# sriramelango/optimized-diffusion-model

Hardware: AMD Instinct MI355X
Metric: trajectories/sec (1000-step PC sampler, NCSN++ [1,9,9], bs=128/GPU) (higher is better)
Workload: dtype f32; 1 GPU; NCSN++ nf=64 ch_mult=[1,2,2] on [128,1,9,9] per GPU, 1000-step reflected PC sampler (predictor euler_maruyama, corrector none), classifier-free guidance on (2B-sample forwards), fp32; global_batch=128, num_scales=1000, score_evals_per_traj=999, parallelism=single GPU

## Files before the change

### optimized-diffusion-model_amd/csrc/rdmi.hip

```cpp
#include <hip/hip_runtime.h>

#include <algorithm>
#include <cmath>
#include <cstdarg>
#include <cstdio>
#include <cstdlib>
#include <cstring>
#include <climits>
#include <map>
#include <memory>
#include <stdexcept>
#include <string>
#include <vector>

#include "../../include/rdmi.h"
#include "attn_kernel.h"
#include "conv_kernel.h"
#include "misc_kernels.h"
#include "unet_kernel.h"
#include "bwd_kernels.h"
#include "opt_kernels.h"
#include "ode_kernels.h"
#include "tiled_kernels.h"

// ... 270 lines not shown
    }
    add_conv_p(c, "input_conv", a.channels, a.nf);
    for (auto& b : L.down) add_resblock_p(c, b.name, b.cin, b.cout);
    for (size_t i = 0; i < L.down.size(); ++i)
        if (L.down[i].attn) add_attn_p(c, "down_attn." + std::to_string(i), L.down[i].cout);
    {
        int ch = a.nf;
        for (int i = 0; i < a.n_levels; ++i) {
            ch = a.nf * a.ch_mult[i];
            if (i != a.n_levels - 1) add_conv_p(c, "downsample." + std::to_string(i) + ".Conv_0", ch, ch);
        }
    }
    add_resblock_p(c, "mid_block1", L.mid_ch, L.mid_ch);
    add_resblock_p(c, "mid_block2", L.mid_ch, L.mid_ch);
    for (auto& b : L.up) add_resblock_p(c, b.name, b.cin, b.cout);
    for (size_t i = 0; i < L.up.size(); ++i)
        if (L.up[i].attn) add_attn_p(c, "up_attn." + std::to_string(i), L.up[i].cout);
    for (int k = 0, i = a.n_levels - 1; i >= 1; --i, ++k) {
        const int ch = a.nf * a.ch_mult[i];
        add_conv_p(c, "upsample." + std::to_string(k) + ".Conv_0", ch, ch);
    }
    add_gn(c, "out_norm", a.nf * a.ch_mult[0]);
    add_conv_p(c, "out_conv", a.nf * a.ch_mult[0], a.channels);
}

inline bool up_fold_shape_ok(int Hs, int Ws, int Cin, int Cout) {
    return std::getenv("RDMI_NO_UP_FOLD") == nullptr && Hs * Ws == 16 && Cin == Cout && Cin % 128 == 0;
}

inline bool k_fold_shape_ok(int C, int L) {
    return std::getenv("RDMI_NO_K_FOLD") == nullptr && std::getenv("RDMI_NO_ATTN_FOLD") == nullptr && std::getenv("RDMI_NO_QKV1") == nullptr && C == 64 && L <= 96;
}

struct Builder {
    rdmi_ctx* c;
    std::vector<int> ints;
    size_t wf = 0;

    int new_tensor(const std::string& name, int C, int H, int W) {
        Tensor t;
        t.name = name; t.C = C; t.H = H; t.W = W;
        t.def = (int)c->ops.size();
        c->tensors.push_back(t);
        return (int)c->tensors.size() - 1;
    }
    void use(int t) { if (t >= 0) c->tensors[t].last = (int)c->ops.size(); }

    size_t alloc_w(size_t n) { size_t o = wf; wf += (n + 63) & ~(size_t)63; return o; }

    void job_pack(const std::string& pname, size_t dst_off, int Cin, int Cout, int Kpad, int Npad, int n_off, int ntap,
                  long s_co, long s_ci, long s_t) {
        PackJob j{};
        j.dst = reinterpret_cast<float*>(dst_off);
        j.Cin = Cin; j.Cout = Cout; j.Kpad = Kpad; j.Npad = Npad; j.n_off = n_off; j.ntap = ntap;
        j.s_co = s_co; j.s_ci = s_ci; j.s_t = s_t; j.kind = 0;
        c->jobs.push_back(j);
        c->job_param.push_back(c->pindex.at(pname));
    }
    void job_copy(const std::string& pname, size_t dst_off, int n, int n_off) {
        PackJob j{};
        j.dst = reinterpret_cast<float*>(dst_off);
        j.Cout = n; j.n_off = n_off; j.kind = 1;
        c->jobs.push_back(j);
        c->job_param.push_back(c->pindex.at(pname));
    }
    size_t pack_conv(const std::string& pre, int cin, int cout) {
// ... 600 lines not shown
            const BlockSpec& bs = L.up[u];
            HS sk = hs.back();
            hs.pop_back();
            const int Hs = H, Ws = W;
            H = sk.H; W = sk.W;
            h = add_resblock(b, bs.name, h, sk.t, ch, sk.C, Hs, Ws, H, W, bs.cout, dense_off[bs.name], &err);
            if (err) return err;
            ch = bs.cout;
            if (bs.attn) { h = b.add_attn("up_attn." + std::to_string(u), h, ch, H, W, &err); if (err) return err; }
        }
        if (k != a.n_levels - 1) {
            ConvSpec s;
            s.name = "upsample." + std::to_string(k);
            s.tA = h; s.CA = ch; s.Ha = H; s.Wa = W; s.Hv = 2 * H; s.Wv = 2 * W;
            s.conv = s.name + ".Conv_0"; s.Ho = 2 * H; s.Wo = 2 * W; s.Cout = ch;
            h = b.add_conv(s, &err);
            if (err) return err;
            if (k == a.n_levels - 2 && up_fold_shape_ok(H, W, ch, ch)) {
                const int Kp = pad16(ch), Np = pad16(ch);
                const size_t o = b.alloc_w((size_t)16 * Kp * Np);
                b.job_pack(s.conv + ".weight", o, ch, ch, Kp, Np, 0, 16, (long)ch * 9, 9, 1);
                c->jobs.back().kind = 5;
                c->wmap[s.conv + ".up4"] = o;
            }
            H *= 2; W *= 2;
        }
    }
    if (H != c->H || W != c->W) return fail("network output grid %dx%d != input %dx%d", H, W, c->H, c->W);
    ConvSpec out;
    out.name = "out_conv"; out.tA = h; out.CA = ch; out.Ha = H; out.Wa = W; out.Hv = H; out.Wv = W;
    out.gn = "out_norm"; out.conv = "out_conv"; out.Ho = H; out.Wo = W; out.Cout = a.channels; out.to_output = true;
    b.add_conv(out, &err);
    if (err) return err;

    {
        struct Blk { size_t off, size; };
        std::vector<Blk> freel;
        std::vector<std::vector<int>> dies((size_t)c->ops.size() + 1);
        for (size_t t = 0; t < c->tensors.size(); ++t) {
            Tensor& tt = c->tensors[t];
            if (tt.last < tt.def) tt.last = tt.def;
            dies[(size_t)tt.last].push_back((int)t);
        }
        size_t top = 0;
        size_t ti = 0;
        for (size_t o = 0; o < c->ops.size(); ++o) {
            for (; ti < c->tensors.size() && c->tensors[ti].def == (int)o; ++ti) {
                Tensor& tt = c->tensors[ti];
                const size_t need = (tt.per_sample() + 63) & ~(size_t)63;
                int best = -1;
                if (!c->debug_taps)
                    for (size_t f = 0; f < freel.size(); ++f)
                        if (freel[f].size >= need && (best < 0 || freel[f].size < freel[(size_t)best].size)) best = (int)f;
                if (best >= 0) {
                    tt.off = freel[(size_t)best].off;
                    if (freel[(size_t)best].size > need) { freel[(size_t)best].off += need; freel[(size_t)best].size -= need; }
                    else freel.erase(freel.begin() + best);
                } else { tt.off = top; top += need; }
            }
            for (int t : dies[o]) {
                const Tensor& tt = c->tensors[(size_t)t];
                freel.push_back({tt.off, (tt.per_sample() + 63) & ~(size_t)63});
            }
        }
        c->ws_per_sample = top;
    }
// ... 155 lines not shown
        for (int p = 0; p < 4; ++p)
            for (int y = 0; y < Hs; ++y)
                for (int x = 0; x < Ws; ++x) {
                    const int sy = y + (tap >> 1) - 1 + (p >> 1), sx = x + (tap & 1) - 1 + (p & 1);
                    if (sy >= 0 && sy < Hs && sx >= 0 && sx < Ws) v[(size_t)p * Hs * Ws + y * Ws + x] = (short)(sy * Ws + sx);
                }
        char key[64];
        snprintf(key, sizeof key, "up4:%d,%d,%d", Hs, Ws, tap);
        return add_table(key, v);
    }

    FOp blank(int kind) {
        FOp o;
        std::memset(&o, 0, sizeof o);
        o.kind = kind; o.a_off = -1; o.b_off = -1; o.a_map_off = -1; o.dense_off = -1; o.resid_off = -1; o.scale = 1.f; o.src_off = -1; o.gn_off = -1; o.samp = cur_samp; o.drop_op = -1;
        return o;
    }
    int emit(const FOp& o) { flush_xchg(); prog.fprog.push_back(o); return (int)prog.fprog.size() - 1; }
    int emit_xchg(const LT& t, const LT* own_rows_src) {
        FOp o = blank(FOP_XCHG);
        o.dst_off = t.off; o.dst_rs = t.rs; o.xidx = n_xchg++;
        if (own_rows_src) {
            o.a_hw = 1; o.rows = own_rows_src->hw(); o.C = t.C; o.a_off = own_rows_src->off; o.a_rs = own_rows_src->rs;
            if (own_rows_src->C != t.C || t.rows() != 4 * o.rows) fail_("exchange: row-slice shapes");
        } else {
            o.a_hw = 0; o.rows = t.rows(); o.C = t.C / 4;
        }
        if (o.C < 32 || o.C > 128 || (o.C & (o.C - 1)) || o.rows * o.C > 512) fail_("exchange: block of " + std::to_string(o.rows) + " x " + std::to_string(o.C));
        xslot_granules = std::max(xslot_granules, 2 * o.rows * o.C);
        prog.fprog.push_back(o);
        return (int)prog.fprog.size() - 1;
    }
    void flush_xchg() { if (pendx.on) { pendx.on = false; emit_xchg(pendx.t, nullptr); } }
    enum { F_GAMMA, F_BETA, F_BIAS, F_BIAS2, F_W, F_SC0W, F_SC1W, F_BIAS_ARENA };
    void patch_param(int op, int field, const std::string& param) { prog.fpatch.push_back({op, field, param, 0}); }
    void patch_arena(int op, int field, size_t off) { prog.fpatch.push_back({op, field, "", off}); }

    void gather_x(const LT& dst) {
        FOp o = blank(FOP_GATHER);
        o.dst_off = dst.off; o.dst_rs = dst.rs; o.rows = dst.rows(); o.C = dst.C;
        o.CA = c->arch.channels; o.CB = 0; o.a_off = -2; o.a_hw = dst.hw(); o.hw_shift = shift_of(dst.hw());
        emit(o);
    }
    void gather_g(const LT& dst, size_t spill) {
        FOp o = blank(FOP_GATHER);
        o.dst_off = dst.off; o.dst_rs = dst.rs; o.rows = dst.rows(); o.C = dst.C;
        o.CA = dst.C; o.CB = 0; o.a_off = -1; o.a_hw = dst.hw(); o.a_mod = 0; o.hw_shift = shift_of(dst.hw());
        const int idx = emit(o);
        spill_fix.push_back({idx, spill, 2});
    }
    void gather_cat(const LT& dst, const LT& A, size_t spillB, int CB) {
        FOp o = blank(FOP_GATHER);
        o.dst_off = dst.off; o.dst_rs = dst.rs; o.rows = dst.rows(); o.C = dst.C;
        o.CA = A.C; o.CB = CB; o.a_off = A.off; o.a_rs = A.rs; o.a_hw = A.hw(); o.hw_shift = shift_of(dst.hw());
        if (A.H != dst.H || A.W != dst.W || A.pm) o.a_map_off = map_table(A.H, A.W, dst.H, dst.W, A.pm);
        if (A.pm && A.ns != 1) fail_("phase-major tensors are single-sample");
        o.b_off = -1;
        const int idx = emit(o);
        spill_fix.push_back({idx, spillB, 1});
    }
    void copy_t(const LT& dst, const LT& src) {
        if (src.pm) fail_("copy of a phase-major tensor");
        FOp o = blank(FOP_GATHER);
        o.dst_off = dst.off; o.dst_rs = dst.rs; o.rows = dst.rows(); o.C = dst.C;
        o.CA = src.C; o.CB = 0; o.a_off = src.off; o.a_rs = src.rs; o.a_hw = src.hw(); o.hw_shift = shift_of(dst.hw());
        emit(o);
    }
    struct SpillFix { int op; size_t off; int which; };
    std::vector<size_t> slot_log; size_t slot_pos = 0; bool slot_replay = false;
    std::vector<SpillFix> spill_fix;
    size_t spill_store(const LT& t) {
        if (t.pm) fail_("spill of a phase-major tensor");
        FOp o = blank(FOP_STORE);
        o.dst_off = t.off; o.dst_rs = t.rs; o.rows = t.rows(); o.C = t.C; o.hw_shift = shift_of(t.hw());
// ... 110 lines not shown
                }
            }
            prog.fprog[(size_t)idx].drop_op = -1;
        }
        if (coop && cur_samp < 0) {
            FOp& q = prog.fprog[(size_t)idx];
            q.coop = 1;
            if (q.Cout_pad != 128 || q.mtiles != 1 || q.main_ph.nch % 4 != 0 || dst_kind != 0 || !dst || dst->C != 128)
                fail_("co-operative conv shape (Cout " + std::to_string(Cout) + ", " + std::to_string(q.mtiles) + " row tiles, " + std::to_string(q.main_ph.nch) + " chunks)");
            if (ntap == 9) { pendx.on = true; pendx.t = *dst; }
        }
        return idx;
    }
    bool up_fold_ok(const LT& in, int Hv, int Wv, int Cout) const {
        return !train && cur_samp >= 0 && !in.pm && Hv == 2 * in.H && Wv == 2 * in.W && up_fold_shape_ok(in.H, in.W, in.C, Cout) &&
               c->wmap.count("upsample." + std::to_string(c->arch.n_levels - 2) + ".Conv_0.up4") != 0;
    }
    int conv_up4(const LT& in, const std::string& wkey, int Cout, const std::string& bias_param, LT* dst) {
        FOp o = blank(FOP_CONV);
        o.rows = 4 * in.hw(); o.mtiles = 4; o.Cout = Cout; o.Cout_pad = pad16(Cout);
        o.ntap = 4; o.hw_shift = shift_of(o.rows);
        o.main_ph.lds_off = in.off; o.main_ph.rs = in.rs; o.main_ph.nch = in.C / 16;
        for (int t = 0; t < 4; ++t) o.tab_off[t] = up4_table(in.H, in.W, t);
        o.w_tile_stride = 4 * in.C * o.Cout_pad * (int)sizeof(float);
        o.dst_off = dst->off; o.dst_rs = dst->rs;
        if (o.main_ph.nch % 8 != 0 || o.rows <= 4 || o.dst_kind != 0 || in.C != Cout || in.hw() != 16 || in.pm || cur_samp < 0 || dst->C != Cout || dst->hw() != o.rows)
            fail_("folded upsample conv: unsupported shape (" + std::to_string(in.H) + "x" + std::to_string(in.W) + " source, " + std::to_string(in.C) + " -> " + std::to_string(Cout) + " channels)");
        dst->pm = true;
        const int idx = emit(o);
        patch_arena(idx, F_W, c->wmap.at(wkey + ".up4"));
        patch_param(idx, F_BIAS, bias_param);
        return idx;
    }
};

FusedBuilder::LT fused_resblock(FusedBuilder& b, const std::string& name, FusedBuilder::LT& xin, int cout, int dense_off) {
    using LT = FusedBuilder::LT;
    const int H = xin.H, W = xin.W;
    const float rs2 = (float)(1.0 / std::sqrt(2.0));
    if (xin.C != cout) {
        LT out = b.talloc(cout, H, W);
        b.conv(xin, H, W, H, W, 1, 0, 1, name + ".NIN_0", 0, cout, name + ".NIN_0.b", 0, 0, &out, 1.f, -1, nullptr, nullptr, "", "");
        b.gn(xin, name + ".GroupNorm_0", true);
        LT h1 = b.talloc(cout, H, W);
        b.conv(xin, H, W, H, W, 1, 1, 9, name + ".Conv_0", 0, cout, name + ".Conv_0.bias", 0, 0, &h1, 1.f, dense_off, nullptr, nullptr, "", "");
        b.tfree(xin);
        b.gn(h1, name + ".GroupNorm_1", true);
        b.conv(h1, H, W, H, W, 1, 1, 9, name + ".Conv_1", 0, cout, name + ".Conv_1.bias", 0, 0, &out, rs2, -1, &out, nullptr, "", "");
        b.tfree(h1);
        return out;
    }
    LT xact = b.talloc(xin.C, H, W);
    b.gn(xact, name + ".GroupNorm_0", true, &xin);
    LT h1 = b.talloc(cout, H, W);
    b.conv(xact, H, W, H, W, 1, 1, 9, name + ".Conv_0", 0, cout, name + ".Conv_0.bias", 0, 0, &h1, 1.f, dense_off, nullptr, nullptr, "", "");
    b.tfree(xact);
    b.gn(h1, name + ".GroupNorm_1", true);
    LT out = b.talloc(cout, H, W);
    b.conv(h1, H, W, H, W, 1, 1, 9, name + ".Conv_1", 0, cout, name + ".Conv_1.bias", 0, 0, &out, rs2, -1, &xin, nullptr, "", "");
    b.tfree(h1);
    b.tfree(xin);
    return out;
}

FusedBuilder::LT fused_attn(FusedBuilder& b, const std::string& name, FusedBuilder::LT& x) {
    using LT = FusedBuilder::LT;
// ... 93 lines not shown
        for (size_t i = 0; i < c->ops.size(); ++i) b.lp_op[c->ops[i].name] = (int)i;
    }
    const int nslot0 = coop ? 1 : S;
    Layout L = build_layout(c);
    std::map<std::string, int> dense_off;
    {
        int dt = 0;
        for (auto& d : L.down) { dense_off[d.name] = dt; dt += d.cout; }
        dense_off["mid_block1"] = dt; dt += L.mid_ch;
        dense_off["mid_block2"] = dt; dt += L.mid_ch;
        for (auto& u : L.up) { dense_off[u.name] = dt; dt += u.cout; }
    }
    const int zero_bytes = 1280;
    const int stat_bytes = 1024 + 64;
    b.arena_init(TAB_RESERVE + zero_bytes + stat_bytes);
    b.gn_slot_off = TAB_RESERVE + zero_bytes;
    b.gn_fuse = std::getenv("RDMI_NO_GNFUSE") == nullptr;
    const int H0 = c->H, W0 = c->W;
    if (H0 * W0 > 96) { q.why = "more than 96 pixels per sample"; return 0; }
    const int nlev = a.n_levels;
    const bool multi = S > 1;

    struct HS { size_t spill; int C, H, W; };
    std::vector<HS> hs;
    int ch = a.nf, H = H0, W = W0;
    size_t hand_down = 0, hand_up = 0;
    LT h;
    const int nrb = a.num_res_blocks;
    for (int sl = 0; sl < nslot0; ++sl) {
        b.cur_samp = sl;
        b.slot_replay = sl > 0; b.slot_pos = 0;
        H = H0; W = W0; ch = a.nf;
        LT xin = b.talloc(16, H, W);
        b.gather_x(xin);
        h = b.talloc(a.nf, H, W);
        b.conv(xin, H, W, H, W, 1, 1, 9, "input_conv", 0, a.nf, "input_conv.bias", 0, 0, &h, 1.f, -1, nullptr, nullptr, "", "");
        b.tfree(xin);
        if (sl == 0) hs.push_back({(size_t)-1, a.nf, H, W});
        for (int j = 0; j < nrb; ++j) {
            const BlockSpec& bs = L.down[(size_t)j];
            h = fused_resblock(b, bs.name, h, bs.cout, dense_off[bs.name]);
            ch = bs.cout;
            if (bs.attn) h = fused_attn(b, "down_attn." + std::to_string(j), h);
            const size_t sp = b.spill_store(h);
            if (sl == 0) hs.push_back({sp, ch, H, W});
        }
        if (sl == 0) hs.push_back(hs.back());
        if (nlev > 1) {
            const int Ho = (H + 1 - 3) / 2 + 1, Wo = (W + 1 - 3) / 2 + 1;
            LT o = b.talloc(ch, Ho, Wo);
            const std::string nm = "downsample.0.Conv_0";
            b.conv(h, H, W, Ho, Wo, 2, 0, 9, nm, 0, ch, nm + ".bias", 0, 0, &o, 1.f, -1, nullptr, nullptr, "", "");
            b.tfree(h);
            h = o; H = Ho; W = Wo;
            if (multi && !coop) { hand_down = b.spill_store(h); b.tfree(h); }
        }
    }
    b.slot_replay = false;
    int d = nrb, u = 0, loadtab_idx = -1;
    {
        b.cur_samp = (multi && !coop) ? -1 : 0;
        int loadtab_op = -1;
        bool in_coop = false;
        auto enter_multi = [&]() {
            b.multi_slot_off = b.alloc_top(4096);
            b.tab1_lds = b.alloc_top(TAB1_RESERVE);
            FOp lt = b.blank(FOP_LOADTAB);
            lt.dst_off = b.tab1_lds;
            loadtab_op = b.emit(lt);
// ... 78 lines not shown
        if (multi && !coop) {
            hand_up = b.spill_store(h); b.tfree(h);
            leave_multi();
        }
        loadtab_idx = loadtab_op;
    }
    const int u0 = u, ch_low = ch, H_low = H, W_low = W;
    const std::vector<HS> hs0 = hs;
    for (int sl = 0; sl < nslot0; ++sl) {
        b.cur_samp = sl;
        u = u0; ch = ch_low; H = H_low; W = W_low; hs = hs0;
        if (multi && !coop) { h = b.talloc(ch, H, W); b.gather_g(h, hand_up); }
        if (nlev > 1) {
            LT o = b.talloc(ch, 2 * H, 2 * W);
            const std::string nm = "upsample." + std::to_string(nlev - 2) + ".Conv_0";
            if (b.up_fold_ok(h, 2 * H, 2 * W, ch)) b.conv_up4(h, nm, ch, nm + ".bias", &o);
            else b.conv(h, 2 * H, 2 * W, 2 * H, 2 * W, 1, 1, 9, nm, 0, ch, nm + ".bias", 0, 0, &o, 1.f, -1, nullptr, nullptr, "", "");
            b.tfree(h);
            h = o; H *= 2; W *= 2;
        }
        for (int j = 0; j < nrb + 1; ++j, ++u) {
            const BlockSpec& bs = L.up[(size_t)u];
            HS sk = hs.back();
            hs.pop_back();
            LT cat = b.talloc(ch + sk.C, sk.H, sk.W);
            b.gather_cat(cat, h, sk.spill, sk.C);
            b.tfree(h);
            H = sk.H; W = sk.W;
            h = fused_resblock(b, bs.name, cat, bs.cout, dense_off[bs.name]);
            ch = bs.cout;
            if (bs.attn) h = fused_attn(b, "up_attn." + std::to_string(u), h);
        }
        b.gn(h, "out_norm", true);
        b.conv(h, H, W, H, W, 1, 1, 9, "out_conv", 0, a.channels, "out_conv.bias", 0, 2, nullptr, 1.f, -1, nullptr, nullptr, "", "");
        b.tfree(h);
    }
    if (H != c->H || W != c->W) b.fail_("network output grid differs from the input grid");

    *tab_used = (int)q.ftabs.size() * 2 + 16;
    *tab1_used = (int)b.tabs1.size() * 2 + 16;
    if (*tab_used > TAB_RESERVE && TAB_RESERVE != 8 * 1024) b.fail_("row tables exceed the reserved LDS region");
    if (*tab1_used > TAB1_RESERVE && multi) b.fail_("low-resolution row tables exceed their LDS block");
    int cmax = 16;
    for (auto& o : q.fprog) if (o.kind == FOP_CONV) { cmax = std::max(cmax, o.main_ph.nch * 16); for (int s2 = 0; s2 < o.nsc; ++s2) cmax = std::max(cmax, o.sc[s2].nch * 16); }
    if (cmax * 4 + 64 > zero_bytes) b.fail_("zero row too small");
    if (b.failed && TAB_RESERVE == 8 * 1024 && *tab_used <= 8 * 1024) return 0;
    if (b.failed) { q.why = b.why; return 0; }

    auto tab_lds = [&](int ref) { return (ref >> 24) ? b.tab1_lds + (ref & 0xffffff) * 2 : (ref & 0xffffff) * 2; };
    for (auto& o : q.fprog) {
        if (o.kind == FOP_CONV) {
            for (int t = 0; t < o.ntap; ++t) o.tab_off[t] = tab_lds(o.tab_off[t]);
            for (int s2 = 0; s2 < o.nsc; ++s2) o.sc[s2].tab_off = tab_lds(o.sc[s2].tab_off);
        } else if (o.kind == FOP_GATHER && o.a_map_off >= 0) {
            o.a_map_off = tab_lds(o.a_map_off);
        }
    }
    while (q.ftabs.size() % 8) q.ftabs.push_back(-1);
    const size_t tab0_shorts = q.ftabs.size();
    q.ftabs.insert(q.ftabs.end(), b.tabs1.begin(), b.tabs1.end());
    q.spill_per_sample = b.spill_floats;
    int coop_max_nb = 0, spill_n = c->max_batch;
    if (coop) {
        const int st = c->coop_stride, res = resident_workgroups();
        const int max_groups = (res / (4 * st)) * st;
        coop_max_nb = std::min(c->max_batch, 4 * max_groups);
        if (coop_max_nb < 1) b.fail_("no room for one co-operative group");
        const int grid_max = ceil_div(ceil_div(std::max(coop_max_nb, 1), 4), st) * 4 * st;
        spill_n = 4 * grid_max;
    }
    if (b.failed) { q.why = b.why; return 0; }
    HIP_OK(hip_alloc(q.d_spill, std::max<size_t>(q.spill_per_sample, 1) * (size_t)spill_n));
    HIP_OK(hip_alloc(q.d_fprog, q.fprog.size()));
    HIP_OK(hip_alloc(q.d_ftabs, q.ftabs.size()));
    HIP_OK(hipMemcpy(q.d_ftabs.get(), q.ftabs.data(), q.ftabs.size() * sizeof(short), hipMemcpyHostToDevice));
    for (auto& f : b.spill_fix) {
        FOp& o = q.fprog[(size_t)f.op];
        float* p = q.d_spill.get() + f.off * (size_t)spill_n;
        if (f.which == 1) o.b_g = p; else if (f.which == 2) o.a_g = p; else o.g_out = p;
    }
    UnetArgs& fa = q.fargs;
    fa = UnetArgs{};
    fa.prog = q.d_fprog.get(); fa.nops = (int)q.fprog.size();
    fa.tabs = q.d_ftabs.get(); fa.tab_bytes = (int)(tab0_shorts * sizeof(short)); fa.tab_base = 0;
    if (loadtab_idx >= 0) q.fprog[(size_t)loadtab_idx].a_g = reinterpret_cast<const float*>(q.d_ftabs.get() + tab0_shorts);
    fa.zero_off = TAB_RESERVE; fa.zero_bytes = zero_bytes;
// ... 129 lines not shown
    }
    HIP_OK(hipGetLastError());
    for (auto& op : c->ops) {
        if (op.kind == OP_CONV) {
            ConvArgs& a = op.conv;
            a.bias = P(c, op.p_bias);
            a.bias_sc = op.p_bias_sc.empty() ? nullptr : P(c, op.p_bias_sc);
            a.gamma = op.p_gamma.empty() ? nullptr : P(c, op.p_gamma);
            a.beta = op.p_beta.empty() ? nullptr : P(c, op.p_beta);
        } else {
            op.attn.gamma = P(c, op.p_gamma); op.attn.beta = P(c, op.p_beta); op.attn.b3 = P(c, op.p_b3);
        }
    }
    for (auto& l : c->tl) {
        if (l.kind == 6) { l.gact.gamma = P(c, l.p_gamma); l.gact.beta = P(c, l.p_beta); continue; }
        if (l.kind != 0) continue;
        l.conv.bias = l.p_bias.empty() ? c->d_w.get() + l.bias_arena : P(c, l.p_bias);
        l.conv.gamma = l.p_gamma.empty() ? nullptr : P(c, l.p_gamma);
        l.conv.beta = l.p_beta.empty() ? nullptr : P(c, l.p_beta);
    }
    for (auto& q : c->progs) {
        if (!q.ok) continue;
        for (auto& f : q.fpatch) {
            FOp& o = q.fprog[(size_t)f.op];
            const float* p = f.param.empty() ? c->d_w.get() + f.arena_off : P(c, f.param);
            switch (f.field) {
                case FusedBuilder::F_GAMMA: o.gamma = p; break;
                case FusedBuilder::F_BETA: o.beta = p; break;
                case FusedBuilder::F_BIAS: case FusedBuilder::F_BIAS_ARENA: o.bias = p; break;
                case FusedBuilder::F_BIAS2: o.bias2 = p; break;
                case FusedBuilder::F_W: o.main_ph.w = p; break;
                case FusedBuilder::F_SC0W: o.sc[0].w = p; break;
                case FusedBuilder::F_SC1W: o.sc[1].w = p; break;
            }
        }
        HIP_OK(hipMemcpyAsync(q.d_fprog.get(), q.fprog.data(), q.fprog.size() * sizeof(FOp), hipMemcpyHostToDevice, s));
    }
    if (c->fused_ready()) HIP_OK(hipStreamSynchronize(s));
    c->packed_valid = true;
    return 0;
}

struct FwdIn {
    const float* x; int x_mod;
    const float* sig; int sig_mod;
    float t_scalar;
    int t_is_time; float smin, ratio;
    const float* labels; int label_rows;
    float* out; int NB;
    const float* tt_row = nullptr;
    const float* dense_rows = nullptr;
};

int run_forward(rdmi_ctx* c, const FwdIn& f, hipStream_t s) {
    const rdmi_arch& a = c->arch;
    if (f.NB < 1 || f.NB > c->max_batch) return fail("batch %d outside [1, %d] (rdmi_create max_batch)", f.NB, c->max_batch);
    if (a.scale_by_sigma && !c->tiled) return fail("scale_by_sigma=True is only built for the tiled plan (the shipped GTO-Halo config sets it False, RD/configs/model/ncsnpp.yaml)");
    if (a.conditional && !f.labels) return fail("class_labels is required: the model is conditional (label_emb) -- reference raises here too (RD/models/ncsnpp.py:262)");
    const int T = c->temb, Np_t = (T + 63) & ~63, Np_d = (c->dense_total + 63) & ~63;
    if (!f.tt_row && !f.dense_rows) {
    LinArgs l{};
    l.M = f.NB; l.fourW = P(c, "time_embed.W"); l.nfour = a.nf;
    l.X = f.sig; l.x_mod = f.sig_mod > 0 ? f.sig_mod : f.NB; l.t_is_time = f.t_is_time; l.smin = f.smin; l.ratio = f.ratio;
    l.use_scalar = f.sig ? 0 : 1; l.t_scalar = f.t_scalar;
    l.pre = 2; l.K = pad16(2 * a.nf); l.W = c->d_w.get() + c->w_t0; l.Npad = Np_t; l.N = T; l.bias = P(c, "time_mlp.0.bias");
    l.Y = c->d_h1.get(); l.ldy = T;
// ... 862 lines not shown
```

### optimized-diffusion-model_amd/csrc/unet_kernel.h

```cpp
#pragma once
#include <cstddef>

#include "common.h"

#define UW_THREADS 512
#define UW_WAVES 8
#ifndef UW_PF_M4
#define UW_PF_M4 4
#endif
#ifndef UW_PF_N1
#define UW_PF_N1 4
#endif
#ifndef UW_PF_KS1
#define UW_PF_KS1 4
#endif
#ifndef UW_PRIO
#define UW_PRIO 0
#endif
#ifndef UW_LIGHT_BARRIER
#define UW_LIGHT_BARRIER 0
#endif

__device__ __forceinline__ void lds_barrier() {
#if defined(__HIP_DEVICE_COMPILE__) && UW_LIGHT_BARRIER
// ... 19 lines not shown
    int CA, CB;
    int a_off, a_rs, a_hw, a_mod, a_map_off;
    int b_off, b_rs;
    const float* a_g; const float* b_g;
    float* g_out;
    int G, act; float eps;
    int src_off, src_rs;
    int logT, Cg, magic_c4n, magic_Cg; float inv_cnt;
    int logG;
    const float* gamma; const float* beta;
    int ntap; int tab_off[9];
    FPhase main_ph;
    int nsc; FPhase sc[2];
    int mtiles, Cout, Cout_pad;
    const float* bias; const float* bias2;
    int dense_off;
    int resid_off, resid_rs;
    float scale;
    int dst_kind;
    int dst2_off, dst3_off, dst3_rs, split_C;
    int q_off, k_off, vt_off, p_off, qk_rs, ps;
    int L, Lpad; float att_scale;
    int gn_off, gn_rs, gn_act, gn_raw, gn_slot_off, gn_nslots;
    int samp, hw_shift;
    int qkv1;
    int coop;
    int a_mstride;
    int xidx;
    float* stash;
    int stash_bf16;
    int drop_op;
    int w_tile_stride;
    int k_rs;
};

struct UnetArgs {
    const FOp* prog; int nops;
    const short* tabs; int tab_bytes;
    int tab_base;
    int zero_off;
    int zero_bytes;
    const float* dense; int dense_stride;
    const float* x_in; int x_mod;
    float* out;
    int NB;
    int S;
    int dbg;
    long long* stamps;
    int coop, coop_stride;
    unsigned long long* xbuf;
    int xslot;
    unsigned epoch_base;
    int out_elems;
    float drop_p; const unsigned long long* seed_dev;
    int* coop_err;
    int coop_break;
};

struct OpW { int w0, w1; };
static_assert(sizeof(FOp) <= 512, "FOp must fit two VGPRs per wave");
__device__ __forceinline__ int opw_at(const OpW& r, int word) {
    return word < 64 ? __builtin_amdgcn_readlane(r.w0, word) : __builtin_amdgcn_readlane(r.w1, word - 64);
}
#define OPI(r, field) opw_at(r, (int)(offsetof(FOp, field) / 4))
#define OPF(r, field) __builtin_bit_cast(float, OPI(r, field))
#define OPP(r, T, field) \
    reinterpret_cast<T*>((unsigned long long)(unsigned)opw_at(r, (int)(offsetof(FOp, field) / 4)) | ((unsigned long long)(unsigned)opw_at(r, (int)(offsetof(FOp, field) / 4) + 1) << 32))
__device__ __forceinline__ OpW opw_load(const FOp* op, int lane) {
    OpW r;
    constexpr int NW = (int)(sizeof(FOp) / 4);
    const int* g = reinterpret_cast<const int*>(op);
    r.w0 = lane < NW ? __builtin_bit_cast(int, ldg1(reinterpret_cast<const float*>(g + lane))) : 0;
    r.w1 = lane + 64 < NW ? __builtin_bit_cast(int, ldg1(reinterpret_cast<const float*>(g + lane + 64))) : 0;
    return r;
}

__device__ __forceinline__ float* lds_f(int off) { return reinterpret_cast<float*>(rdmi_lds + off); }

__device__ __forceinline__ int samp_of(int samp, int hw_shift, int row) { return samp >= 0 ? samp : (row >> hw_shift); }

template <bool MS>
__device__ __forceinline__ void fop_gather(const OpW& w, const UnetArgs& u, int n0, int ncap, int member, int tid) {
    struct { int C, rows, dst_off, dst_rs, CA, CB, a_off, a_rs, a_hw, a_mod, a_map_off, b_off, b_rs, samp, hw_shift; const float* a_g; const float* b_g; } o;
    o.C = OPI(w, C); o.rows = OPI(w, rows); o.dst_off = OPI(w, dst_off); o.dst_rs = OPI(w, dst_rs); o.CA = OPI(w, CA); o.CB = OPI(w, CB);
    o.a_off = OPI(w, a_off); o.a_rs = OPI(w, a_rs); o.a_hw = OPI(w, a_hw); o.a_mod = OPI(w, a_mod); o.a_map_off = OPI(w, a_map_off);
    if (MS && o.a_off >= 0) o.a_off += member * OPI(w, a_mstride);
    o.b_off = OPI(w, b_off); o.b_rs = OPI(w, b_rs); o.a_g = OPP(w, const float, a_g); o.b_g = OPP(w, const float, b_g);
    o.samp = MS ? OPI(w, samp) : 0; o.hw_shift = MS ? OPI(w, hw_shift) : 0;
    const int Cd = o.C;
    const int c4n = Cd >> 2;
    const int total = o.rows * c4n;
    float* dst = lds_f(o.dst_off);
    const short* map = o.a_map_off >= 0 ? reinterpret_cast<const short*>(rdmi_lds + o.a_map_off) : nullptr;
    const int dpv = UW_THREADS / c4n, dc4 = UW_THREADS - dpv * c4n;
    int row = tid / c4n, c4 = tid - row * c4n;
    const bool from_x = o.a_off == -2;
    const float* ag = from_x ? u.x_in : o.a_g;
    const int amod = from_x ? u.x_mod : o.a_mod;
    const int hw = o.samp >= 0 ? o.rows : (1 << o.hw_shift);
    for (int i = tid; i < total; i += UW_THREADS) {
        const int c = c4 << 2;
        const int sl = samp_of(o.samp, o.hw_shift, row);
        const int px = o.samp >= 0 ? row : row - (sl << o.hw_shift);
        const int n = min(n0 + sl, ncap - 1);
        f32x4 val = {0.f, 0.f, 0.f, 0.f};
        if (c < o.CA) {
            const int srow = map ? map[px] : px;
            if (o.a_off >= 0) {
                val = *reinterpret_cast<const f32x4*>(lds_f(o.a_off) + (size_t)((o.samp >= 0 ? 0 : sl * o.a_hw) + srow) * o.a_rs + c);
            } else {
                const int nA = amod > 0 ? n % amod : n;
                const float* p = ag + ((size_t)nA * o.a_hw + srow) * o.CA + c;
                if ((o.CA & 3) == 0) val = ldg4(p);
                else
                    for (int j = 0; j < 4; ++j)
                        if (c + j < o.CA) val[j] = ldg1(p + j);
            }
        } else if (c < o.CA + o.CB) {
            if (o.b_off >= 0) val = *reinterpret_cast<const f32x4*>(lds_f(o.b_off) + (size_t)row * o.b_rs + (c - o.CA));
            else val = ldg4(o.b_g + ((size_t)n * hw + px) * o.CB + (c - o.CA));
        }
        *reinterpret_cast<f32x4*>(dst + (size_t)row * o.dst_rs + c) = val;
        row += dpv; c4 += dc4;
        if (c4 >= c4n) { c4 -= c4n; ++row; }
    }
}

template <bool MS>
__device__ __forceinline__ void fop_store(const OpW& w, const UnetArgs& u, int n0, int ncap, int tid) {
    struct { int C, rows, dst_off, dst_rs, samp, hw_shift; float* g_out; } o;
    o.C = OPI(w, C); o.rows = OPI(w, rows); o.dst_off = OPI(w, dst_off); o.dst_rs = OPI(w, dst_rs); o.g_out = OPP(w, float, g_out);
    o.samp = MS ? OPI(w, samp) : 0; o.hw_shift = MS ? OPI(w, hw_shift) : 0;
    const int c4n = o.C >> 2;
    const int total = o.rows * c4n;
    const float* src = lds_f(o.dst_off);
    const int hw = o.samp >= 0 ? o.rows : (1 << o.hw_shift);
    const int dpv = UW_THREADS / c4n, dc4 = UW_THREADS - dpv * c4n;
    int row = tid / c4n, c4 = tid - row * c4n;
    for (int i = tid; i < total; i += UW_THREADS) {
        const int sl = samp_of(o.samp, o.hw_shift, row);
        const int px = o.samp >= 0 ? row : row - (sl << o.hw_shift);
        const int n = min(n0 + sl, ncap - 1);
        stg4(o.g_out + ((size_t)n * hw + px) * o.C + (c4 << 2), *reinterpret_cast<const f32x4*>(src + (size_t)row * o.dst_rs + (c4 << 2)));
        row += dpv; c4 += dc4;
        if (c4 >= c4n) { c4 -= c4n; ++row; }
    }
// ... 730 lines not shown
                        else fconv_main<DIAG, 1, UW_PF_M4, true>(w, u, mt0, WM, nt, lane, fine, acc);
                    } else if (tapm8) fconv_main_t<DIAG, 1, false, 8>(w, u, mt0, WM, nt, lane, fine, acc, (unsigned)mt0 * (unsigned)wts);
                    else if (tapm) fconv_main_t<DIAG, 1>(w, u, mt0, WM, nt, lane, fine, acc);
                    else fconv_main<DIAG, 1, UW_PF_N1>(w, u, mt0, WM, nt, lane, fine, acc);
                    break;
                case 2: fconv_main<DIAG, 2, 8>(w, u, mt0, WM, nt, lane, fine, acc); break;
                case 3: {
                    const int last_rows = OPI(w, rows) - (mt0 + 2 * WM) * 16;
                    const bool lm4 = last_rows >= 1 && last_rows <= 4 && OPI(w, dst_kind) != 1 && OPI(w, dst_kind) != 3;
                    if (tapm) { if (lm4) fconv_main_t<DIAG, 3, true>(w, u, mt0, WM, nt, lane, fine, acc); else fconv_main_t<DIAG, 3>(w, u, mt0, WM, nt, lane, fine, acc); }
                    else if (lm4) fconv_main<DIAG, 3, 4, false, true>(w, u, mt0, WM, nt, lane, fine, acc);
                    else fconv_main<DIAG, 3, 4>(w, u, mt0, WM, nt, lane, fine, acc);
                    break;
                }
                case 4:
                    if (tapm) fconv_main_t<DIAG, 4>(w, u, mt0, WM, nt, lane, fine, acc);
                    else fconv_main<DIAG, 4, 4>(w, u, mt0, WM, nt, lane, fine, acc);
                    break;
                default: break;
            }
            if (DIAG && (u.dbg & 256)) continue;
            use_from_here(add1); use_from_here(add2); use_from_here(dv);
            const float add = col < o_Cout ? (o_bias2 ? add1 + add2 : add1) : 0.f, dadd0 = o_dense >= 0 ? dv : 0.f;
            fconv_epi<MS, TR>(w, u, n0, mt0, WM, nt, nmt, lane, add, dadd0, daddm, acc, ps1, ps2);
            k_mt0 = mt0; k_nt = nt; k_nmt = nmt;
            if (DIAG && fine) fine[5] = clock64();
        }
    }
    if (fused_gn) {
        use_from_here(gmul); use_from_here(gadd);
        lds_barrier();
        if (DIAG && fine) fine[6] = clock64();
        if (k_nmt > 0) fconv_gn_apply<MS, TR>(w, u, n0, k_mt0, WM, k_nt, k_nmt, lane, gmul, gadd, acc, ps1, ps2);
        if (DIAG && fine) fine[7] = clock64();
    }
}

template <bool DIAG>
__device__ __forceinline__ void fop_conv_coop(const OpW& w, const UnetArgs& u, int n_grp, int m, int wave, int lane, long long* fine) {
    const int lrow = lane & 15, kq = lane >> 4;
    const int ct = wave & 1, kg = wave >> 1;
    const int nt = 2 * m + ct, col = nt * 16 + lrow;
    const int o_Cout = OPI(w, Cout), o_dense = OPI(w, dense_off), hw_shift = OPI(w, hw_shift);
    const float* o_bias = OPP(w, const float, bias); const float* o_bias2 = OPP(w, const float, bias2);
    const bool fused_gn = OPI(w, gn_off) >= 0;
    const bool finisher = kg == 0;
    float add1 = ldg1(o_bias + col), add2 = ldg1((o_bias2 ? o_bias2 : o_bias) + col);
    float gmul = ldg1((fused_gn ? OPP(w, const float, gamma) : o_bias) + col), gadd = ldg1((fused_gn ? OPP(w, const float, beta) : o_bias) + col);
    float dv = ldg1(u.dense + (size_t)max(o_dense, 0) + (o_dense >= 0 ? (size_t)min(n_grp + ((kq * 4) >> hw_shift), u.NB - 1) * u.dense_stride + col : 0));
    f32x4 acc[4];
    {
        const int spt = OPI(w, main_ph.nch) >> 2;
        if (spt == 2) fconv_main_ks<DIAG, 2>(w, u, nt, lane, fine, acc, kg);
        else if (spt == 4 && (OPI(w, main_ph.nch) & 3) == 0) fconv_main_ks<DIAG, 4>(w, u, nt, lane, fine, acc, kg);
        else fconv_main<DIAG, 1, UW_PF_KS1, false, false, true>(w, u, 0, 1, nt, lane, fine, acc, kg);
    }
    float* const dstp = lds_f(OPI(w, dst_off));
    const int drs = OPI(w, dst_rs);
    if (!finisher) {
        float* p = dstp + (size_t)(kq * 4) * drs + (((m + kg) & 3) * 32 + ct * 16 + lrow);
#pragma unroll
        for (int r = 0; r < 4; ++r) p[r * drs] = acc[0][r];
    }
    use_from_here(add1); use_from_here(add2); use_from_here(dv); use_from_here(gmul); use_from_here(gadd);
    lds_barrier();
    if (finisher) {
// ... 235 lines not shown
    OpW cur = opw_load(u.prog, lane);
    OpW nxt = opw_load(u.prog + (u.nops > 1 ? 1 : 0), lane);
    f32x4 pgm = {1.f, 1.f, 1.f, 1.f}, pbt = {0.f, 0.f, 0.f, 0.f};
    gn_prefetch(cur, tid, pgm, pbt);
    for (int pc = 0; pc < u.nops; ++pc) {
        const OpW nn = opw_load(u.prog + (pc + 2 < u.nops ? pc + 2 : u.nops - 1), lane);
        long long* fine = (DIAG && u.stamps && n == 0 && tid == ((u.dbg >> 16) & 7) * 64) ? u.stamps + 1024 + pc * 8 : nullptr;
        const int kind = OPI(cur, kind);
        if (DIAG && fine) fine[2] = clock64();
        f32x4 ngm = pgm, nbt = pbt;
        if (pc + 1 < u.nops) gn_prefetch(nxt, tid, ngm, nbt);
        if (DIAG && fine) fine[3] = clock64();
        const int skip = (DIAG && u.dbg) ? ((kind == FOP_GN ? 4 : kind == FOP_CONV ? 8 : kind == FOP_ATTN ? 16 : 32) & u.dbg) : 0;
        const bool multi = MS && OPI(cur, samp) < 0;
        switch (skip ? -1 : kind) {
            case FOP_GATHER: fop_gather<MS>(cur, u, multi ? n_spill : n, multi ? spill_cap : u.NB, COOP ? cm : 0, tid); break;
            case FOP_STORE: fop_store<MS>(cur, u, multi ? n_spill : n, multi ? spill_cap : u.NB, tid); break;
            case FOP_GN: fop_gn<MS>(cur, stat, tid, pgm, pbt, DIAG ? u.dbg : 0); break;
            case FOP_CONV:
                if (COOP && OPI(cur, coop)) fop_conv_coop<DIAG>(cur, u, n_multi, cm, wave, lane, fine);
                else fop_conv<DIAG, MS && !COOP, TRAIN>(cur, u, multi ? n_multi : n, wave, lane, fine);
                break;
            case FOP_ATTN: fop_attn(cur, wave, lane); break;
            case FOP_LOADTAB: {
                const int* src = OPP(cur, const int, a_g);
                int* dst = reinterpret_cast<int*>(rdmi_lds + OPI(cur, dst_off));
                const int nw = OPI(cur, rows) >> 2;
                for (int i = tid; i < nw; i += UW_THREADS) dst[i] = src[i];
                break;
            }
            case FOP_XCHG: if (COOP) fop_xchg(cur, u, cg, cm, tid, failw); break;
            default: break;
        }
        if (kind == FOP_STORE || (kind == FOP_CONV && OPI(cur, dst_kind) == 2)) __syncthreads();
        else lds_barrier();
        if (DIAG && u.stamps && n == 0 && tid == 0) u.stamps[pc + 1] = clock64();
        cur = nxt; nxt = nn; pgm = ngm; pbt = nbt;
    }
    if (COOP && *failw) {
        const int E = (int)u.out_elems;
        for (int i = tid; i < E; i += UW_THREADS) u.out[(size_t)n * E + i] = __builtin_nanf("");
    }
}
```

Before: 185.6 trajectories/s.

## Fold single-channel input/output 3x3 convs into dense 9-tap GEMMs

For the one-channel input, the input conv now gathers its 9 taps im2col-style into 16 columns and runs as a 1-tap conv with K=16, instead of a 9-tap conv over a channel dimension padded to 16. The output conv is done the other way round: a 1x1 GEMM writes 9 per-tap partial outputs, then a per-pixel tap-sum epilogue adds the shifted partials plus the bias and writes to global memory. This removes the padding waste where 9 taps each multiplied mostly-zero 16-wide channel blocks. It adds packed weights, an extra LDS buffer and a full __syncthreads after the tap-sum op.

```diff
diff --git a/optimized-diffusion-model_amd/csrc/rdmi.hip b/optimized-diffusion-model_amd/csrc/rdmi.hip
--- a/optimized-diffusion-model_amd/csrc/rdmi.hip
+++ b/optimized-diffusion-model_amd/csrc/rdmi.hip
@@ -326,6 +326,10 @@
     return std::getenv("RDMI_NO_K_FOLD") == nullptr && std::getenv("RDMI_NO_ATTN_FOLD") == nullptr && std::getenv("RDMI_NO_QKV1") == nullptr && C == 64 && L <= 96;
 }
 
+inline bool io_fold_shape_ok(int channels) {
+    return std::getenv("RDMI_NO_IO_FOLD") == nullptr && channels >= 1 && 9 * channels <= 16;
+}
+
 struct Builder {
     rdmi_ctx* c;
     std::vector<int> ints;
@@ -992,6 +996,16 @@
     out.gn = "out_norm"; out.conv = "out_conv"; out.Ho = H; out.Wo = W; out.Cout = a.channels; out.to_output = true;
     b.add_conv(out, &err);
     if (err) return err;
+    if (io_fold_shape_ok(a.channels)) {
+        const int K9 = 9 * a.channels;
+        const size_t oi = b.alloc_w((size_t)16 * pad16(a.nf));
+        b.job_pack("input_conv.weight", oi, K9, a.nf, 16, pad16(a.nf), 0, 1, K9, 1, 0);
+        c->wmap["input_conv.d9"] = oi;
+        const int Kp = pad16(ch);
+        const size_t oo = b.alloc_w((size_t)Kp * 16 + 16);
+        b.job_pack("out_conv.weight", oo, ch, K9, Kp, 16, 0, 1, 1, 9, 0);
+        c->wmap["out_conv.t9"] = oo;
+    }
 
     {
         struct Blk { size_t off, size; };
@@ -1213,14 +1227,31 @@
         return (int)prog.fprog.size() - 1;
     }
     void flush_xchg() { if (pendx.on) { pendx.on = false; emit_xchg(pendx.t, nullptr); } }
-    enum { F_GAMMA, F_BETA, F_BIAS, F_BIAS2, F_W, F_SC0W, F_SC1W, F_BIAS_ARENA };
+    enum { F_GAMMA, F_BETA, F_BIAS, F_BIAS2, F_W, F_SC0W, F_SC1W, F_BIAS_ARENA, F_TSUM_BIAS };
     void patch_param(int op, int field, const std::string& param) { prog.fpatch.push_back({op, field, param, 0}); }
     void patch_arena(int op, int field, size_t off) { prog.fpatch.push_back({op, field, "", off}); }
 
-    void gather_x(const LT& dst) {
+    bool io_fold_ok() const {
+        return !train && io_fold_shape_ok(c->arch.channels) && c->wmap.count("input_conv.d9") != 0 && c->wmap.count("out_conv.t9") != 0;
+    }
+    void tap9_tables(int H, int W, int* first, int* step) {
+        int t[9];
+        for (int k = 0; k < 9; ++k) t[k] = tap_table(H, W, H, W, H, W, 1, 1, k);
+        for (int k = 2; k < 9; ++k)
+            if (t[k] - t[k - 1] != t[1] - t[0] || (t[k] >> 24) != (t[0] >> 24)) fail_("dense input / output conv: tap tables not evenly spaced");
+        *first = t[0]; *step = t[1] - t[0];
+    }
+    void gather_x(const LT& dst, bool im2col = false) {
         FOp o = blank(FOP_GATHER);
         o.dst_off = dst.off; o.dst_rs = dst.rs; o.rows = dst.rows(); o.C = dst.C;
         o.CA = c->arch.channels; o.CB = 0; o.a_off = -2; o.a_hw = dst.hw(); o.hw_shift = shift_of(dst.hw());
+        if (im2col) {
+            if (cur_samp < 0 || dst.ns != 1 || dst.C != 16 || c->arch.channels != 1) fail_("dense input conv: one channel, one sample per op");
+            int step = 0;
+            o.ntap = o.CA = 9;
+            tap9_tables(dst.H, dst.W, &o.tab_off[0], &step);
+            o.tab_off[1] = o.tab_off[0] + step;
+        }
         emit(o);
     }
     void gather_g(const LT& dst, size_t spill) {
@@ -1397,6 +1428,19 @@
         patch_param(idx, F_BIAS, bias_param);
         return idx;
     }
+    int conv_tapsum(const LT& in, const std::string& bias_param, const LT* dst) {
+        const int K9 = 9 * c->arch.channels;
+        if (cur_samp < 0 || in.ns != 1 || c->arch.channels != 1 || dst->C < K9 || dst->hw() != in.hw() || in.hw() > UW_THREADS)
+            fail_("dense output conv: one channel, one sample per op");
+        const int idx = conv(in, in.H, in.W, in.H, in.W, 1, 1, 1, "out_conv.t9", 0, K9, "", c->wmap.at("out_conv.t9") + (size_t)pad16(in.C) * 16, 0, dst, 1.f, -1,
+                             nullptr, nullptr, "", "");
+        int first = 0, step = 0;
+        tap9_tables(in.H, in.W, &first, &step);
+        FOp& q = prog.fprog[(size_t)idx];
+        q.tsum = 9; q.tsum_tab = first; q.tsum_ts = step;
+        patch_param(idx, F_TSUM_BIAS, bias_param);
+        return idx;
+    }
 };
 
 FusedBuilder::LT fused_resblock(FusedBuilder& b, const std::string& name, FusedBuilder::LT& xin, int cout, int dense_off) {
@@ -1556,9 +1600,10 @@
         b.slot_replay = sl > 0; b.slot_pos = 0;
         H = H0; W = W0; ch = a.nf;
         LT xin = b.talloc(16, H, W);
-        b.gather_x(xin);
+        const bool io_fold = b.io_fold_ok();
+        b.gather_x(xin, io_fold);
         h = b.talloc(a.nf, H, W);
-        b.conv(xin, H, W, H, W, 1, 1, 9, "input_conv", 0, a.nf, "input_conv.bias", 0, 0, &h, 1.f, -1, nullptr, nullptr, "", "");
+        b.conv(xin, H, W, H, W, 1, 1, io_fold ? 1 : 9, io_fold ? "input_conv.d9" : "input_conv", 0, a.nf, "input_conv.bias", 0, 0, &h, 1.f, -1, nullptr, nullptr, "", "");
         b.tfree(xin);
         if (sl == 0) hs.push_back({(size_t)-1, a.nf, H, W});
         for (int j = 0; j < nrb; ++j) {
@@ -1703,7 +1748,11 @@
             if (bs.attn) h = fused_attn(b, "up_attn." + std::to_string(u), h);
         }
         b.gn(h, "out_norm", true);
-        b.conv(h, H, W, H, W, 1, 1, 9, "out_conv", 0, a.channels, "out_conv.bias", 0, 2, nullptr, 1.f, -1, nullptr, nullptr, "", "");
+        if (b.io_fold_ok()) {
+            LT p9 = b.talloc(16, H, W);
+            b.conv_tapsum(h, "out_conv.bias", &p9);
+            b.tfree(p9);
+        } else b.conv(h, H, W, H, W, 1, 1, 9, "out_conv", 0, a.channels, "out_conv.bias", 0, 2, nullptr, 1.f, -1, nullptr, nullptr, "", "");
         b.tfree(h);
     }
     if (H != c->H || W != c->W) b.fail_("network output grid differs from the input grid");
@@ -1723,6 +1772,9 @@
         if (o.kind == FOP_CONV) {
             for (int t = 0; t < o.ntap; ++t) o.tab_off[t] = tab_lds(o.tab_off[t]);
             for (int s2 = 0; s2 < o.nsc; ++s2) o.sc[s2].tab_off = tab_lds(o.sc[s2].tab_off);
+            if (o.tsum) { o.tsum_ts = tab_lds(o.tsum_tab + o.tsum_ts) - tab_lds(o.tsum_tab); o.tsum_tab = tab_lds(o.tsum_tab); }
+        } else if (o.kind == FOP_GATHER && o.ntap) {
+            for (int t = 0; t < 2; ++t) o.tab_off[t] = tab_lds(o.tab_off[t]);
         } else if (o.kind == FOP_GATHER && o.a_map_off >= 0) {
             o.a_map_off = tab_lds(o.a_map_off);
         }
@@ -1918,6 +1970,7 @@
                 case FusedBuilder::F_W: o.main_ph.w = p; break;
                 case FusedBuilder::F_SC0W: o.sc[0].w = p; break;
                 case FusedBuilder::F_SC1W: o.sc[1].w = p; break;
+                case FusedBuilder::F_TSUM_BIAS: o.tsum_bias = p; break;
             }
         }
         HIP_OK(hipMemcpyAsync(q.d_fprog.get(), q.fprog.data(), q.fprog.size() * sizeof(FOp), hipMemcpyHostToDevice, s));
diff --git a/optimized-diffusion-model_amd/csrc/unet_kernel.h b/optimized-diffusion-model_amd/csrc/unet_kernel.h
--- a/optimized-diffusion-model_amd/csrc/unet_kernel.h
+++ b/optimized-diffusion-model_amd/csrc/unet_kernel.h
@@ -75,6 +75,8 @@
     int drop_op;
     int w_tile_stride;
     int k_rs;
+    const float* tsum_bias;
+    int tsum, tsum_tab, tsum_ts;
 };
 
 struct UnetArgs {
@@ -141,6 +143,7 @@
     const float* ag = from_x ? u.x_in : o.a_g;
     const int amod = from_x ? u.x_mod : o.a_mod;
     const int hw = o.samp >= 0 ? o.rows : (1 << o.hw_shift);
+    const int ntap = OPI(w, ntap), tap0 = opw_at(w, (int)(offsetof(FOp, tab_off) / 4)), tap_step = opw_at(w, (int)(offsetof(FOp, tab_off) / 4) + 1) - tap0;
     for (int i = tid; i < total; i += UW_THREADS) {
         const int c = c4 << 2;
         const int sl = samp_of(o.samp, o.hw_shift, row);
@@ -154,7 +157,13 @@
             } else {
                 const int nA = amod > 0 ? n % amod : n;
                 const float* p = ag + ((size_t)nA * o.a_hw + srow) * o.CA + c;
-                if ((o.CA & 3) == 0) val = ldg4(p);
+                if (ntap) {
+                    p = ag + (size_t)nA * o.a_hw;
+                    for (int j = 0; j < 4; ++j) {
+                        const int s = c + j < ntap ? (int)*reinterpret_cast<const short*>(rdmi_lds + tap0 + (c + j) * tap_step + px * 2) : -1;
+                        if (s >= 0) val[j] = ldg1(p + s);
+                    }
+                } else if ((o.CA & 3) == 0) val = ldg4(p);
                 else
                     for (int j = 0; j < 4; ++j)
                         if (c + j < o.CA) val[j] = ldg1(p + j);
@@ -951,6 +960,26 @@
         lds_barrier();
         if (DIAG && fine) fine[6] = clock64();
         if (k_nmt > 0) fconv_gn_apply<MS, TR>(w, u, n0, k_mt0, WM, k_nt, k_nmt, lane, gmul, gadd, acc, ps1, ps2);
+        if (DIAG && fine) fine[7] = clock64();
+    }
+    if (const int ntaps = OPI(w, tsum)) {
+        const int rows = OPI(w, rows), rs = OPI(w, dst_rs), t0 = OPI(w, tsum_tab), ts = OPI(w, tsum_ts), row = wave * 64 + lane;
+        const float* const P = lds_f(OPI(w, dst_off));
+        float* const g_dst = OPP(w, float, g_out) ? OPP(w, float, g_out) : u.out;
+        float b = ldg1(OPP(w, const float, tsum_bias));
+        lds_barrier();
+        if (DIAG && fine) fine[6] = clock64();
+        if (row < rows) {
+            float sum = 0.f;
+#pragma unroll 1
+            for (int t = 0; t < ntaps; ++t) {
+                const int s = *reinterpret_cast<const short*>(rdmi_lds + t0 + t * ts + row * 2);
+                const float v = P[max(s, 0) * rs + t];
+                sum += s >= 0 ? v : 0.f;
+            }
+            use_from_here(b);
+            stg1(g_dst + (size_t)min(n0 + max(o_samp, 0), u.NB - 1) * rows + row, sum + b);
+        }
         if (DIAG && fine) fine[7] = clock64();
     }
 }
@@ -1252,7 +1281,7 @@
             case FOP_XCHG: if (COOP) fop_xchg(cur, u, cg, cm, tid, failw); break;
             default: break;
         }
-        if (kind == FOP_STORE || (kind == FOP_CONV && OPI(cur, dst_kind) == 2)) __syncthreads();
+        if (kind == FOP_STORE || (kind == FOP_CONV && (OPI(cur, dst_kind) == 2 || OPI(cur, tsum)))) __syncthreads();
         else lds_barrier();
         if (DIAG && u.stamps && n == 0 && tid == 0) u.stamps[pc + 1] = clock64();
         cur = nxt; nxt = nn; pgm = ngm; pbt = nbt;
```

After: 186.9 trajectories/s (median of 6 runs). No clear change (+0.7%).
